# nauful/NLZM

Hardware: AMD Instinct MI355X
Metric: compress MB/s (higher is better)
Workload: dtype u8; 1 GPU; enwik9 stand-in: 1000000000 B stream, -window:28; step = 41 launches of 8 chunks (40136704 B) of the stream; timed: bytes [200683520, 401367040) of 1000000000 (a prefix: the steps asked for end before the stream does); window_bits=28, batch_chunks=8, whole_stream=False

## Files before the change

nlzm_amd/csrc/nlzm_hip.cpp:

```cpp
#include <hip/hip_runtime.h>
#include <dirent.h>
#include <unistd.h>

#include <stdarg.h>
#include <stdint.h>
#include <stdio.h>
#include <stdlib.h>
#include <string.h>

#include <array>
#include <mutex>
#include <thread>
#include <chrono>
#include <algorithm>
#include <vector>

#include "../../include/nlzm_hip.h"
#include "nlzm_core.h"
#include "nlzm_v2.h"

namespace nlzm {
void launch_rk_hash(const uint8_t *in, unsigned long long n, unsigned long long pos0, unsigned long long pos1,
                    uint32_t *out, hipStream_t st);
void launch_pipeline2(const Geom &g, const Globals &G, const v2::GlobalsV2 &V, uint32_t c0, uint32_t c1, uint32_t worker_blocks, hipStream_t st);
// ... 653 lines not shown
    if (finished) *finished = C.next_chunk >= g.nchunks;
    return 0;
}

void stage_report(const Persist &P)
{
    const double n = (double)(P.cnt.positions ? P.cnt.positions : 1);
    fprintf(stderr, "cycles/position  finder: total %.0f wait %.0f (%.0f of it for worker results) | table: total %.0f wait %.0f | parser: total %.0f wait %.0f (block set-up %.0f, passes %.0f, emit %.0f)\n",
            P.prof[17] / n, P.prof[16] / n, P.prof[25] / n, P.prof[19] / n, P.prof[18] / n, P.prof[21] / n, P.prof[20] / n, P.prof[23] / n, P.prof[24] / n, P.prof[22] / n);
    fprintf(stderr, "finder: %llu blocks (%.1f positions each); cut by: nice %llu, new top entry %llu, RK candidate %llu, RK catch-up %llu, same worker bin %llu, other %llu\n",
            P.prof[0], n / (double)(P.prof[0] ? P.prof[0] : 1), P.prof[1], P.prof[2], P.prof[3], P.prof[4], P.prof[12], P.prof[5]);
    fprintf(stderr, "table: %llu blocks, %llu on the slow path; parser: %llu blocks (%.1f nodes each), %.2f passes per block (%.0f cycles per pass), mask fills %llu, probe rounds %llu, re-sampled %llu\n",
            P.prof[6], P.prof[7], P.prof[8], n / (double)(P.prof[8] ? P.prof[8] : 1), (double)P.prof[13] / (double)(P.prof[8] ? P.prof[8] : 1),
            (double)P.prof[24] / (double)(P.prof[13] ? P.prof[13] : 1), P.prof[9], P.prof[10], P.prof[11]);
    fprintf(stderr, "table: %llu launches with %u-entry fronts on %u waves (the others: %u on %u), the shape changed %llu times\n", P.prof[114], v2::kFrCapWide, v2::kTWWide, v2::kFrCap, v2::kTW, P.prof[113]);
    fprintf(stderr, "table: blocks in which some position's front had more than 8 / 12 / 16 / 20 / 24 / the launch's capacity of entries at some step of the scan: %.2f / %.2f / %.2f / %.3f / %.3f / %.3f %%\n",
            100.0 * P.prof[105] / (P.prof[6] ? P.prof[6] : 1), 100.0 * P.prof[106] / (P.prof[6] ? P.prof[6] : 1), 100.0 * P.prof[107] / (P.prof[6] ? P.prof[6] : 1),
            100.0 * P.prof[108] / (P.prof[6] ? P.prof[6] : 1), 100.0 * P.prof[109] / (P.prof[6] ? P.prof[6] : 1), 100.0 * P.prof[7] / (P.prof[6] ? P.prof[6] : 1));
    fprintf(stderr, "finder: RK256 entries cut short by the uint16 length parameter that became the growing top entry: %llu; that ended exactly where another entry ends: %llu (%llu of them the nearer one)\n",
            P.prof[115], P.prof[116], P.prof[117]);
    fprintf(stderr, "finder: starts of nice regions whose segment the stage knew itself, ahead of the parser's word: %llu; that it had to wait for: %llu\n", P.prof[118], P.prof[119]);
    fprintf(stderr, "finder: worker results not there at the first look: %llu of positions whose call is the finder's decision (unc), %llu of others\n", P.prof[28], P.prof[29]);
    fprintf(stderr, "finder: blocks that had to wait for a worker result: %llu (%.0f cycles each); late results of hot bins' waves %llu, late results at lane 0 (the position the block before was cut at) %llu\n",
            P.prof[112], (double)P.prof[25] / (double)(P.prof[112] ? P.prof[112] : 1), P.prof[110], P.prof[111]);
    fprintf(stderr, "parser: waited for its record loader %llu times, the table stage %.0f positions ahead on average then\n", P.prof[26], (double)P.prof[27] / (double)(P.prof[26] ? P.prof[26] : 1));
    if (P.prof[96] || P.prof[100])
        fprintf(stderr, "helper parser: %llu jobs posted, %llu taken over (%llu nodes = %.1f %% of the positions), the parser stage waited %.0f cycles per position for it; "
                        "helper: %llu jobs seen, %llu done, %llu blocks (%.2f passes each), waited %.0f cycles per position for records\n",
                P.prof[96], P.prof[97], P.prof[98], 100.0 * P.prof[98] / n, P.prof[99] / n, P.prof[100], P.prof[101], P.prof[102],
                (double)P.prof[103] / (double)(P.prof[102] ? P.prof[102] : 1), P.prof[104] / n);
    if (P.prof[88]) fprintf(stderr, "finder sections (cycles/position, profile build): predict %.0f, own loads %.0f, HT rows %.0f, candidates + jobs %.0f, record + RK256 %.0f, "
                            "BT4 results (wait included) %.0f, verify %.0f, commit %.0f\n", P.prof[88] / n, P.prof[89] / n, P.prof[90] / n, P.prof[91] / n, P.prof[92] / n,
                            P.prof[93] / n, P.prof[94] / n, P.prof[95] / n);
    if (P.prof[44]) fprintf(stderr, "table stage sections (cycles/position summed over the waves, profile build): gather %.0f, scan %.0f, waiting for the carry %.0f, carry merge (the part in block order) %.0f, records %.0f\n",
                            P.prof[44] / n, P.prof[45] / n, P.prof[47] / n, P.prof[46] / n, P.prof[55] / n);
    if (P.prof[32]) {
        const double np = (double)(P.prof[13] ? P.prof[13] : 1);
        fprintf(stderr, "parser, cycles per pass (profile build): relax waves %.0f %.0f %.0f, probe wave %.0f (of it: sets that changed %.0f, mask fills %.0f), update %.0f, "
                        "barrier waits per wave %.0f %.0f %.0f %.0f; block end %.0f cycles/position\n",
                P.prof[32] / np, P.prof[33] / np, P.prof[34] / np, P.prof[35] / np, P.prof[43] / np, P.prof[41] / np, P.prof[40] / np,
                P.prof[36] / np, P.prof[37] / np, P.prof[38] / np, P.prof[39] / np, P.prof[42] / n);
        fprintf(stderr, "parser, cycles per pass by wave 0..7 (profile build): work");
        for (int w = 0; w < 8; w++) fprintf(stderr, " %.0f", P.prof[64 + w] / np);
        fprintf(stderr, " | barrier wait");
        for (int w = 0; w < 8; w++) fprintf(stderr, " %.0f", P.prof[72 + w] / np);
        fprintf(stderr, " | update");
        for (int w = 0; w < 8; w++) fprintf(stderr, " %.0f", P.prof[80 + w] / np);
        fprintf(stderr, "\n");
        const double nbk = (double)(P.prof[8] ? P.prof[8] : 1);
        fprintf(stderr, "parser loader wave, cycles per block set-up: block size + barrier %.0f, re-list %.0f, own edges %.0f, all edges %.0f, literal scan + clear + barrier %.0f\n",
                P.prof[56] / nbk, P.prof[57] / nbk, P.prof[58] / nbk, P.prof[59] / nbk, P.prof[60] / nbk);
        fprintf(stderr, "parser wave 0, cycles per pass: relax %.0f, probe %.0f, clear %.0f | update: keys + cost scan %.0f, membership %.0f, winner sets %.0f, rest %.0f\n",
                P.prof[48] / np, P.prof[49] / np, P.prof[50] / np, P.prof[51] / np, P.prof[52] / np, P.prof[53] / np, P.prof[54] / np);
    }
}
void worker_report(const WorkerCounters &wc, bool hot)
{
    fprintf(stderr, "worker lanes: %llu calls made with their fate open (at and behind a position not decided yet), %llu decisions that took calls back, %llu calls made again for it\n",
            wc.dry_runs, wc.spec_calls, wc.spec_good);
    if (hot)
        fprintf(stderr, "hot bins (a wave each): %llu over all launches, %llu of %llu calls made by their waves\n", wc.hot_bins, wc.hot_calls, wc.bt_calls);
    if (hot && wc.hot_steps) {
            fprintf(stderr, "hot bins' waves: %llu steps (%.1f per call); the next call could not start in %.1f %% of them (a call without its stores on its way) + %.1f %% (an assumed \"skip\" behind a \"call\" still open); lanes: %llu turns spent waiting for a decision\n",
                    wc.hot_steps, (double)wc.hot_steps / (wc.hot_calls ? wc.hot_calls : 1), 100.0 * wc.hot_blocked_dry / wc.hot_steps, 100.0 * wc.hot_blocked_risky / wc.hot_steps, wc.flag_waits);
        fprintf(stderr, "hot bins' waves by the bin's positions in the launch (class: waves | calls, tests/call, entries skipped | steps, cycles/step; the profile build adds | %% of the steps: some lane tests "
                        "(tests per such step; lane-steps repeated for a held slot per step), taking back, every lane holds a call, next call may not start, no entry | idle steps with an undecided position open)\n");
// ... 1064 lines not shown
```

nlzm_amd/csrc/nlzm_v2.h:

```cpp
#pragma once

#include "nlzm_core.h"
#include "xw.h"

namespace nlzm {
namespace v2 {

constexpr uint32_t kFtRing = 1u << 14;
constexpr uint32_t kFtStride = 16;
constexpr uint32_t kTpRing = 1u << 13;
constexpr uint32_t kMaxEdges = 32;
constexpr uint32_t kTpStride = 2 + 2 + 2 * kMaxEdges;
constexpr uint32_t kTpUniq = 2, kTpEdges = 4;
constexpr uint32_t kFrontMax = 264;
constexpr uint32_t kTfStride = 2 * kFrontMax;

constexpr uint32_t kFtBt = 8u, kFtTop = 16u;
struct Hx {
    alignas(128) uint32_t f_pos;
    alignas(128) uint32_t t_pos;
    alignas(128) uint32_t t_out;
    alignas(128) uint32_t p_pos;
    alignas(128) unsigned long long p_seg;
    alignas(128) uint32_t h_job;
// ... 92 lines not shown
#ifndef NLZM_SIM
            if (xw::clock100() - t0 > 3000000000ull) {
                if (xw::lane() == 0) raise(hx, kErrTimeout * 100 + code, code == 1 ? kStFinder : (code <= 3 ? kStTable : kStParser), code, v, xw::ld_agent(w));
                return false;
            }
#else
            (void)t0; (void)code;
#endif
        }
        xw::pause();
    }
}

struct FLds {
    uint32_t ht2[4096];
    uint32_t ht3[16384 + 8];
    uint32_t stage[64 * kFtStride];
    uint32_t job[64 * 3 * 4];
    uint32_t job_len[64 * 4];
    uint32_t njobs;
    uint32_t last[8192];
    Counters cnt;
};

struct Finder {
    Geom g;
    Globals G;
    GlobalsV2 V;
    uint32_t base;
    uint32_t reach;
    uint32_t reach_d = kNone;
    uint32_t s_active, s_d, s_end, s_seen;
    uint32_t rk_from, rk_to, rk_len, rk_end;
    uint32_t rk_cut = 0;
    uint32_t prev_nice, seg_s;
    uint32_t gap_last = 0;
    uint32_t n_seg_own = 0, n_seg_wait = 0;
    uint32_t t_pos_seen;
    uint32_t err;
    uint32_t dbg_a = 0;
    unsigned long long n_pos, n_nice, n_unc, n_ht, n_rkp, n_rki, n_cmp, n_blocks, n_cut0, n_cut1, n_cut2, n_cut3, n_cut4, n_cut5;
    unsigned long long n_cmp_lane = 0;
    unsigned long long t_wait, t_wait_bt = 0, t_total;
    uint32_t n_so_top = 0, n_so_tie = 0, n_so_won = 0;
    uint32_t n_late_unc = 0, n_late_other = 0, n_late_hot = 0, n_late_first = 0, n_late_blocks = 0;
    unsigned long long t_f[8] = {};
#ifdef NLZM_PROFILE
    XW_FN unsigned long long ptick() const { return xw::tick(); }
#else
    XW_FN unsigned long long ptick() const { return 0; }
#endif

    XW_FN void fail(uint32_t code, uint32_t pos, uint32_t site = 0, uint32_t x0 = 0, uint32_t x1 = 0)
    {
        err = code;
        if (xw::lane() == 0) raise(V.hx, code, kStFinder, site, pos, x0, x1);
    }

    uint32_t pend_fpos = 0;
    uint32_t pf_a0 = kNone, pf_rkh = 0;
    unsigned long long pf_own0 = 0, pf_own1 = 0;
    uint8_t pf_unc = 0;
    XW_FN void flush_fpos()
    {
        if (!pend_fpos) return;
        xw::drain();
        if (xw::lane() == 0) xw::st_agent(&V.hx->f_pos, pend_fpos);
        pend_fpos = 0;
    }

    XW_FN void slider_look(uint32_t limit)
    {
        while (s_end == kNone && s_seen < limit) {
            const uint32_t cap = umin(limit - s_seen, 512u);
            const uint32_t l = wave_cmp(G.in, s_seen - s_d, s_seen, 0, cap);
            if (l < cap) s_end = s_seen + l; else s_seen += cap;
        }
        if (s_end == kNone && (unsigned long long)s_seen >= g.n) s_end = (uint32_t)g.n;
    }
// ... 31 lines not shown
                    const uint32_t sa = (uint32_t)(ps >> 32), cover = (uint32_t)ps;
                    const bool covered = (int32_t)(cover - (a0 + 1)) >= 0;
                    const bool own = !covered && (int32_t)(gap_last - cover) < 0 && a0 - sa < kParseMax;
                    if (covered || own) {
                        xw::after_poll();
                        seg_s = sa;
                        n_seg_own += own; n_seg_wait += spins != 0;
                        xw::trace(1, a0, seg_s, (uint32_t)ps);
                        break;
                    }
                    if ((++spins & 63u) == 0) {
                        if (xw::readfirst(xw::ld_agent(&V.hx->err))) { err = kErrInternal + 100; return 1; }
#ifndef NLZM_SIM
                        if (xw::clock100() - t0 > 3000000000ull) { fail(kErrTimeout, a0, 5, (uint32_t)ps, (uint32_t)(ps >> 32)); return 1; }
#else
                        (void)t0;
#endif
                    }
                    xw::pause();
                }
                t_wait += xw::tick() - tw;
            }
        }
        const bool call_full = in_blk && !nice_pred;
        const bool call_some = call_full || (nice_pred && ((a - seg_s) & 7u) == 0);
        const bool ht_call = call_some && avail >= 4;
        const bool rk_call = call_some && avail >= 256;

        uint32_t cut_rk = 64;
        {
            const unsigned long long rkm = xw::ballot(rk_call);
            if (rkm & 1ull) {
                const uint32_t q0 = a0 - base;
                for (uint32_t e = (rk_end | 255u) + 1; e < q0 + 256; e += 256) {
                    const uint32_t hh = xw::readfirst(G.rkhash[base + e - 256]);
                    if (i == 0) G.rk_table[hh >> g.rk_shift] = q0 | (hh << g.wbits);
                    n_rki++;
                }
                xw::drain();
            }
            const unsigned long long below = rkm & ((1ull << i) - 1);
            const uint32_t prev_end = below ? (a0 + (63u - (uint32_t)__builtin_clzll(below))) - base + 256 : rk_end;
            const bool catch_up = rk_call && i > 0 && ((prev_end | 255u) + 1) < q + 256;
            const unsigned long long cm = xw::ballot(catch_up);
            if (cm) cut_rk = (uint32_t)__builtin_ctzll(cm);
        }

        const unsigned long long f1 = ptick();
        uint32_t v4 = 0;
        unsigned long long own0 = 0, own1 = 0;
        uint32_t rkh = 0;
        bool unc = false;
        if (pf_a0 == a0) {
            if (in_blk) { own0 = pf_own0; own1 = pf_own1; v4 = (uint32_t)own0; }
            rkh = rk_call ? pf_rkh : 0u;
            unc = in_blk && G.workers && pf_unc != 0;
        } else {
            if (in_blk) { own0 = load64u(cur); own1 = load64u(cur + 8); v4 = (uint32_t)own0; }
            rkh = rk_call ? G.rkhash[a] : 0u;
            unc = in_blk && G.workers && G.unc[bi] != 0;
        }
        uint32_t rkv = rk_call ? G.rk_table[rkh >> g.rk_shift] : 0u;
        const bool bt_call = call_full && avail >= 4 && G.workers;

        const unsigned long long f2 = ptick();
        const uint32_t h2 = hash4(v4 & 0xFFFFu), h3 = hash4(v4 & 0xFFFFFFu);
        const uint32_t i2 = h2 >> 20, i3 = h3 >> g.ht3_shift;
        const uint32_t tag2 = h2 & g.tag_mask, tag3 = h3 & g.tag_mask;
        const uint32_t e2 = q | (tag2 << g.wbits), e3 = q | (tag3 << g.wbits);
        uint32_t row2 = 0, r0 = 0, r1 = 0;
        if (ht_call) { row2 = L->ht2[i2]; r0 = L->ht3[i3]; r1 = L->ht3[i3 + 1]; }
        const unsigned long long htm = xw::ballot(ht_call);
        bool later = false;
        {
            uint32_t *last = L->last;
            if (ht_call) { xw::lds_max(&last[i2], i + 1); xw::lds_max(&last[4096 + (i3 & 4095u)], i + 1); }
            xw::wave_sync();
            if (ht_call) later = last[i2] > i + 1 || last[4096 + (i3 & 4095u)] > i + 1 || last[4096 + ((i3 + 1) & 4095u)] > i + 1 || last[4096 + ((i3 - 1) & 4095u)] > i + 1;
            xw::wave_sync();
            if (ht_call) { last[i2] = 0; last[4096 + (i3 & 4095u)] = 0; }
        }
        const unsigned long long dep = xw::ballot(later);
        for (unsigned long long mm = dep; mm; mm &= mm - 1) {
            const uint32_t j = (uint32_t)__builtin_ctzll(mm);
            const uint32_t b2 = xw::readlane(i2, j), b3 = xw::readlane(i3, j);
            const uint32_t x2 = xw::readlane(e2, j), x3 = xw::readlane(e3, j), y0 = xw::readlane(r0, j);
            if (ht_call && i > j) {
                if (i2 == b2) row2 = x2;
                if (i3 == b3) { r0 = x3; r1 = y0; }
                else if (i3 == b3 + 1) r0 = y0;
                else if (i3 + 1 == b3) r1 = x3;
            }
        }

        const unsigned long long f3 = ptick();
        uint32_t cd[4] = { 0, 0, 0, 0 };
        if (ht_call) {
            const uint32_t s0 = row2 & g.wmask, s1 = r0 & g.wmask, s2 = r1 & g.wmask;
            if ((row2 >> g.wbits) == tag2 && s0 < q && q - s0 <= g.wmask) cd[0] = q - s0;
            if ((r0 >> g.wbits) == tag3 && s1 < q && q - s1 <= g.wmask) cd[1] = q - s1;
            if ((r1 >> g.wbits) == tag3 && s2 < q && q - s2 <= g.wmask) cd[2] = q - s2;
        }
        const bool rk_act = rk_len > 0 && q - rk_to < rk_len;
        const uint32_t rk_eff = rk_act ? rk_len : 0u;
        const bool rk_probe = rk_call && rk_eff < 256;
        bool rk_cand = false;
        uint32_t rk_d = 0;
        if (rk_probe) {
            const uint32_t sp = rkv & g.wmask;
            if ((rkv >> g.wbits) == (rkh & g.tag_mask) && sp < q && q - sp <= g.wmask) { rk_cand = true; rk_d = q - sp; }
        }
        uint32_t rk_l16 = 16;
        if (rk_cand) {
            const unsigned long long x0 = load64u(cur - rk_d) ^ own0;
            if (x0) rk_l16 = (uint32_t)__builtin_ctzll(x0) >> 3;
            else {
                const unsigned long long x1 = load64u(cur - rk_d + 8) ^ own1;
                rk_l16 = x1 ? 8 + ((uint32_t)__builtin_ctzll(x1) >> 3) : 16;
            }
        }
        const bool rk_short = rk_cand && rk_l16 < 16 && rk_l16 < (avail & 0xFFFFu);
        const bool rk_dropped = rk_short && !(rk_l16 >= rk_eff && rk_l16 >= match_min(rk_d));
        uint32_t cl[3] = { 0, 0, 0 };
        L->njobs = 0;
        xw::wave_sync();
        unsigned long long cx0[3], cx1[3];
#pragma unroll
        for (int k = 0; k < 3; k++) {
// ... 181 lines not shown
                    so_top = so_free && (so_end > umax(before, ec) || so_win);
                    stm = xw::ballot(so_top);
                    js = stm ? (uint32_t)__builtin_ctzll(stm) : 64u;
                    const unsigned long long bad = xw::ballot(in_blk && nice_real != nice_pred);
                    cut_nice = bad ? (uint32_t)__builtin_ctzll(bad) : 64u;
                    om = xw::ballot(in_blk && od != kNone && (!s_sliding || od < s_d));
                    jo = om ? (uint32_t)__builtin_ctzll(om) : 64u;
                    m = umin(n, umin(cut_nice, umin(jo + 1 > 64 ? 64u : jo + 1, umin(cut_ev, umin(cut_rk, umin(cut_slot, cut_bin))))));
                    m = umin(m, js + 1 > 64 ? 64u : js + 1);
                    if (unc && avail >= 4 && !told && i < umin(F, m)) { xw::st_agent(G.bt_flag + bi, nice_real ? kFlagSkip : kFlagCall); told = true; }
                    if (m <= F) break;
                    if (i == F && unc) xw::st_agent(G.bt_flag + bi, kFlagCall);
                }
                if ((++spins & 63u) == 0) {
                    if (xw::readfirst(xw::ld_agent(&V.hx->err))) { err = kErrInternal + 100; return 1; }
#ifndef NLZM_SIM
                    if (xw::clock100() - t0 > 3000000000ull) {
                        const uint32_t fl = (uint32_t)__builtin_ctzll(missing | (1ull << 63));
                        fail(kErrTimeout, a0 + fl, 6, (uint32_t)__builtin_popcountll(missing) | (xw::readlane(unc ? 1u : 0u, fl) << 8) | (n << 16),
                             xw::readlane((hash4(v4) >> g.bt_shift) % G.nheads, fl));
                        return 1;
                    }
#else
                    (void)t0;
#endif
                }
                xw::pause();
            }
            if (waits) { t_wait += xw::tick() - tw; t_wait_bt += xw::tick() - tw; }
        }

        const unsigned long long f6 = ptick();
        if (m == 0) { fail(kErrInternal, a0, 7); return 1; }
        n_blocks++;
        if (m < n) {
            const uint32_t w = m == cut_nice ? 0u : (m == jo + 1 ? 1u : (m == cut_ev ? 2u : (m == cut_rk ? 3u : (m == cut_bin ? 5u : 4u))));
            n_cut0 += w == 0; n_cut1 += w == 1; n_cut2 += w == 2; n_cut3 += w == 3; n_cut4 += w == 4; n_cut5 += w == 5;
        }
        const bool fin = i < m;
        {
            const unsigned long long gapm = xw::ballot(fin && umax(before, s_sliding ? s_e : 0u) <= a);
            if (gapm) gap_last = a0 + (63u - (uint32_t)__builtin_clzll(gapm));
        }
        if (stm || xw::any(so_tie)) {
            n_so_top += (uint32_t)__builtin_popcountll(xw::ballot(fin && so_top)); n_so_tie += (uint32_t)__builtin_popcountll(xw::ballot(fin && so_tie));
            n_so_won += (uint32_t)__builtin_popcountll(xw::ballot(fin && so_win));
        }

        if (xw::any(fin && nice_real && !unc && avail >= 4 && G.workers)) { fail(kErrV2Promise, a0, 8); return 1; }

        const unsigned long long f7 = ptick();
        for (unsigned long long mm = dep & htm & ((m < 64 ? (1ull << m) : 0ull) - 1ull); mm; mm &= mm - 1) {
            const uint32_t j = (uint32_t)__builtin_ctzll(mm);
            if (i == j) { L->ht2[i2] = e2; L->ht3[i3] = e3; L->ht3[i3 + 1] = r0; }
            xw::wave_sync();
        }
        if (ht_call && i < m && !later) { L->ht2[i2] = e2; L->ht3[i3] = e3; L->ht3[i3 + 1] = r0; }
        xw::wave_sync();
        if (fin && unc && avail >= 4) xw::st_agent(G.bt_flag + bi, nice_real ? kFlagSkip : kFlagCall);
        if (fin && rk_call && (q & 255u) == 0) G.rk_table[rkh >> g.rk_shift] = q | (rkh << g.wbits);
        if (fin) {
            uint32_t w0 = np | (bt_call && bt_n ? kFtBt : 0u) | ((uint32_t)(uint8_t)own0 << 8);
            if (i == jc && s_active && s_end > a + 1) { st[2 + 2 * np] = s_d; st[3 + 2 * np] = s_end - a; np++; w0++; }
            if (s_sliding && i <= jo) { st[14] = s_d; st[15] = cap; w0 |= kFtTop; }
            if (i == jo) { st[14] = od; st[15] = cap; w0 |= kFtTop; }
            st[0] = w0; st[1] = a;
            uint32_t *dst = V.ft + (unsigned long long)(a & (kFtRing - 1)) * kFtStride;
#pragma unroll
            for (int k = 0; k < 4; k++) xw::st_agent128(dst + 4 * k, st[4 * k], st[4 * k + 1], st[4 * k + 2], st[4 * k + 3]);
        }
        {
            const uint32_t last = m - 1;
            const uint32_t pm_last = xw::readlane(pm, last);
            if (pm_last >= reach && pm_last) {
                uint32_t dm = pm_last == reach ? reach_d : kNone;
                const uint32_t le = umax(ec, so_end), ld = umin(ec == le ? ec_d : kNone, so_end == le ? so_d : kNone);
                for (unsigned long long mm = xw::ballot(fin && le == pm_last); mm; mm &= mm - 1) dm = umin(dm, xw::readlane(ld, (uint32_t)__builtin_ctzll(mm)));
                reach = pm_last; reach_d = dm;
            }
            if (s_active && jc <= last) {
                if (s_end > reach) { reach = s_end; reach_d = s_d; } else if (s_end == reach) reach_d = umin(reach_d, s_d);
                s_active = 0;
            }
            if (jo == last) { s_active = 1; s_d = xw::readlane(od, last); s_end = kNone; s_seen = a0 + last + xw::readlane(cap, last); }
            else if (js == last) { s_active = 1; s_d = xw::readlane(so_d, last); s_end = kNone; s_seen = xw::readlane(so_end, last); }
            prev_nice = xw::readlane(nice_real ? 1u : 0u, last);
            const unsigned long long rkf = xw::ballot(fin && rk_call);
            if (rkf) rk_end = (a0 + (63u - (uint32_t)__builtin_clzll(rkf))) - base + 256;
            if (rk_len && xw::any(fin && rk_call && !rk_act)) rk_len = 0;
            if (ev_ok && cut_ev == m) {
                rk_from = (a0 + last - base) - ev_d; rk_to = a0 + last - base; rk_len = ev_l; rk_cut = ev_cut ? 1u : 0u;
            }
        }
        n_pos += m;
        n_nice += (unsigned long long)__builtin_popcountll(xw::ballot(fin && nice_real));
        n_unc += (unsigned long long)__builtin_popcountll(xw::ballot(fin && unc && avail >= 4));
        n_ht += (unsigned long long)__builtin_popcountll(xw::ballot(fin && ht_call));
        n_rkp += (unsigned long long)__builtin_popcountll(xw::ballot(fin && rk_probe));
        n_rki += (unsigned long long)__builtin_popcountll(xw::ballot(fin && rk_call && (q & 255u) == 0));
        n_cmp_lane += fin ? cmpb : 0u;
        pend_fpos = a0 + m;
        pf_a0 = kNone;
        if (a0 + m < a1) {
            pf_a0 = a0 + m;
            const uint32_t na = pf_a0 + i;
            const bool nin = na < a1;
            pf_own0 = nin ? load64u(G.in + na) : 0ull; pf_own1 = nin ? load64u(G.in + na + 8) : 0ull;
            pf_rkh = (nin && la_end - na >= 256) ? G.rkhash[na] : 0u;
            pf_unc = (nin && G.workers) ? G.unc[(unsigned long long)(na - G.batch_a0)] : (uint8_t)0;
        }
        xw::trace(2, a0, n, m, reach, s_active, s_d, s_end);
        {
            const unsigned long long f8 = ptick();
            t_f[0] += f1 - f0; t_f[1] += f2 - f1; t_f[2] += f3 - f2; t_f[3] += f4 - f3; t_f[4] += f5 - f4; t_f[5] += f6 - f5; t_f[6] += f7 - f6; t_f[7] += f8 - f7;
        }
        return m;
    }

    XW_FN void run(uint32_t c0, uint32_t c1)
    {
        FLds *L = xw::lds<FLds>();
        Persist *P = G.persist;
        StateV2 *S = (StateV2 *)V.state;
        const uint32_t i = xw::lane();
        const uint32_t ht3_rows = (1u << (32 - g.ht3_shift)) + 1;
        for (uint32_t k = i; k < 8192; k += 64) L->last[k] = 0;
        for (uint32_t k = i; k < 4096; k += 64) L->ht2[k] = G.ht2[k];
        for (uint32_t k = i; k < ht3_rows; k += 64) L->ht3[k] = G.ht3[k];
        base = xw::readfirst((uint32_t)P->reb_base);
        reach = xw::readfirst(S->reach); reach_d = xw::readfirst(S->reach_d); s_active = xw::readfirst(S->s_active); s_d = xw::readfirst(S->s_d);
        s_end = xw::readfirst(S->s_end); s_seen = xw::readfirst(S->s_seen);
        prev_nice = xw::readfirst(S->prev_nice); seg_s = xw::readfirst(S->seg_s);
        rk_from = xw::readfirst(P->rk_from); rk_to = xw::readfirst(P->rk_to); rk_len = xw::readfirst(P->rk_len); rk_end = xw::readfirst(P->rk_end);
        rk_cut = rk_len >> 31; rk_len &= 0x7FFFFFFFu;
        err = xw::readfirst(P->error);
        if (!err && G.test_fail) fail(kErrInternal + 50, (uint32_t)((unsigned long long)c0 * g.chunk_size), 9);
        n_pos = n_nice = n_unc = n_ht = n_rkp = n_rki = n_cmp = n_blocks = 0;
        n_cut0 = n_cut1 = n_cut2 = n_cut3 = n_cut4 = n_cut5 = 0;
        t_wait = 0;
        const unsigned long long t_start = xw::tick();
        t_pos_seen = (uint32_t)((unsigned long long)c0 * g.chunk_size);
        unsigned long long shifts = 0;
        xw::wave_sync();
        for (uint32_t ci = c0; ci < c1 && !err; ci++) {
            const unsigned long long chunk_abs = (unsigned long long)ci * g.chunk_size;
            const unsigned long long remain = g.n - chunk_abs;
            const uint32_t chunk_read = (uint32_t)(remain < g.feed ? remain : g.feed);
            const uint32_t p_end = umin(g.chunk_size, chunk_read);
            if (chunk_abs - base >= 2ull * (g.wmask + 1)) {
                base += g.wmask + 1;
                shifts++;
                if (i == 0) { L->ht2[0] = kNone; L->ht3[0] = kNone; }
                if (rk_end >= g.wmask + 1) rk_end -= g.wmask + 1; else rk_end = 0;
                xw::wave_sync();
            }
            if (prev_nice) seg_s = (uint32_t)chunk_abs;
            gap_last = (uint32_t)chunk_abs;
            const uint32_t a1 = (uint32_t)chunk_abs + p_end, la_end = (uint32_t)chunk_abs + chunk_read;
            uint32_t a = (uint32_t)chunk_abs;
            while (a < a1 && !err) {
                const uint32_t n = umin(64u, a1 - a);
                dbg_a = a;
                if ((int32_t)(a + n - t_pos_seen - kFtRing) > 0) {
                    flush_fpos();
                    const unsigned long long tw = xw::tick();
                    if (!wait_word_ge(&V.hx->t_pos, a + n - kFtRing, V.hx, 1)) { err = kErrInternal + 100; break; }
                    t_pos_seen = xw::readfirst(xw::ld_agent(&V.hx->t_pos));
                    t_wait += xw::tick() - tw;
                }
                a += block(a, n, a1, la_end);
            }
        }
        flush_fpos();
        for (uint32_t d = 32; d; d >>= 1) n_cmp_lane += xw::shfl64(n_cmp_lane, i ^ d);
        n_cmp += xw::readfirst64(n_cmp_lane);
        xw::wave_sync();
        for (uint32_t k = xw::opaque(i); k < 4096; k += 64) G.ht2[k] = L->ht2[k];
        for (uint32_t k = xw::opaque(i); k < ht3_rows; k += 64) G.ht3[k] = L->ht3[k];
        if (i == 0) {
            P->reb_base = base;
            P->rk_from = rk_from; P->rk_to = rk_to; P->rk_len = rk_len | (rk_cut << 31); P->rk_end = rk_end;
            S->reach = reach; S->reach_d = reach_d; S->s_active = s_active; S->s_d = s_d; S->s_end = s_end; S->s_seen = s_seen;
            S->prev_nice = prev_nice; S->seg_s = seg_s;
            Counters &c = P->cnt;
            xw::atomic_add64_agent(&c.positions, n_pos); xw::atomic_add64_agent(&c.nice_positions, n_nice);
            xw::atomic_add64_agent(&c.uncertain_positions, n_unc); xw::atomic_add64_agent(&c.ht_rows, 3 * n_ht);
            xw::atomic_add64_agent(&c.rk_probes, n_rkp); xw::atomic_add64_agent(&c.rk_inserts, n_rki);
            xw::atomic_add64_agent(&c.cmp_bytes, n_cmp); xw::atomic_add64_agent(&c.shifts, shifts);
            unsigned long long *pr = P->prof;
            xw::atomic_add64_agent(&pr[0], n_blocks); xw::atomic_add64_agent(&pr[1], n_cut0); xw::atomic_add64_agent(&pr[2], n_cut1);
            xw::atomic_add64_agent(&pr[3], n_cut2); xw::atomic_add64_agent(&pr[4], n_cut3); xw::atomic_add64_agent(&pr[5], n_cut4);
            xw::atomic_add64_agent(&pr[12], n_cut5);
            xw::atomic_add64_agent(&pr[16], t_wait); xw::atomic_add64_agent(&pr[17], xw::tick() - t_start); xw::atomic_add64_agent(&pr[25], t_wait_bt);
            xw::atomic_add64_agent(&pr[28], n_late_unc); xw::atomic_add64_agent(&pr[29], n_late_other);
            xw::atomic_add64_agent(&pr[115], n_so_top); xw::atomic_add64_agent(&pr[116], n_so_tie); xw::atomic_add64_agent(&pr[117], n_so_won);
            xw::atomic_add64_agent(&pr[118], n_seg_own); xw::atomic_add64_agent(&pr[119], n_seg_wait);
            xw::atomic_add64_agent(&pr[110], n_late_hot); xw::atomic_add64_agent(&pr[111], n_late_first); xw::atomic_add64_agent(&pr[112], n_late_blocks);
#ifdef NLZM_PROFILE
            for (int z = 0; z < 8; z++) xw::atomic_add64_agent(&pr[88 + z], t_f[z]);
#endif
            if (err || xw::ld_agent(&V.hx->err)) {
                uint32_t *d = V.hx->dbg[0];
                xw::st_agent(d + 0, dbg_a); xw::st_agent(d + 1, reach); xw::st_agent(d + 2, s_active); xw::st_agent(d + 3, s_d);
                xw::st_agent(d + 4, s_end); xw::st_agent(d + 5, prev_nice); xw::st_agent(d + 6, seg_s); xw::st_agent(d + 7, rk_len);
                xw::st_agent(d + 8, t_pos_seen); xw::st_agent(d + 9, err); xw::st_agent(d + 10, base);
            }
        }
    }
};


#ifndef NLZM_FRCAP
#define NLZM_FRCAP 16
#endif
#ifndef NLZM_KTW
#define NLZM_KTW 7
#endif
#ifndef NLZM_FRCAP_WIDE
#define NLZM_FRCAP_WIDE 24
#endif
#ifndef NLZM_KTW_WIDE
#define NLZM_KTW_WIDE 5
#endif
constexpr uint32_t kFrCap = NLZM_FRCAP, kFrCapWide = NLZM_FRCAP_WIDE;
constexpr uint32_t kTW = NLZM_KTW, kTWWide = NLZM_KTW_WIDE;
constexpr uint32_t kTWMax = kTW > kTWWide ? kTW : kTWWide;
constexpr uint32_t kFrArena = (kTW * kFrCap > kTWWide * kFrCapWide ? kTW * kFrCap : kTWWide * kFrCapWide) * 2 * 64;
constexpr uint32_t kTbWidenShift = 6, kTbNarrowShift = 9;
NLZM_HD uint32_t table_waves(uint32_t wide) { return wide ? kTWWide : kTW; }
struct TWave {
    uint32_t recs[64 * kFtStride];
    uint32_t overflow;
// ... 1556 lines not shown
```

nlzm_amd/csrc/xw.h:

```cpp
#pragma once

#include <stdint.h>

#ifndef NLZM_SIM
#include <hip/hip_runtime.h>
#define XW_FN __device__ __forceinline__
#define XW_NOINLINE __device__ __noinline__

namespace xw {

XW_FN uint32_t lane() { return threadIdx.x & 63u; }
XW_FN uint32_t wave() { return (uint32_t)__builtin_amdgcn_readfirstlane((int)(threadIdx.x >> 6)); }
XW_FN uint32_t thread() { return threadIdx.x; }
XW_FN unsigned long long ballot(bool p) { return __ballot(p); }
XW_FN bool any(bool p) { return __ballot(p) != 0; }
XW_FN uint32_t readlane(uint32_t v, uint32_t l) { return (uint32_t)__builtin_amdgcn_readlane((int)v, (int)l); }
XW_FN uint32_t readfirst(uint32_t v) { return (uint32_t)__builtin_amdgcn_readfirstlane((int)v); }
XW_FN unsigned long long readlane64(unsigned long long v, uint32_t l)
{
    return ((unsigned long long)readlane((uint32_t)(v >> 32), l) << 32) | readlane((uint32_t)v, l);
}
XW_FN unsigned long long readfirst64(unsigned long long v)
{
    return ((unsigned long long)readfirst((uint32_t)(v >> 32)) << 32) | readfirst((uint32_t)v);
// ... 62 lines not shown
    u4 v;
    asm volatile("global_load_dwordx4 %0, %1, off sc1\n\ts_waitcnt vmcnt(0)" : "=v"(v) : "v"((const __attribute__((address_space(1))) uint32_t *)p) : "memory");
    return u32x4{ v.x, v.y, v.z, v.w };
}
XW_FN void atomic_or_agent(uint32_t *p, uint32_t v) { (void)__hip_atomic_fetch_or(p, v, __ATOMIC_RELAXED, __HIP_MEMORY_SCOPE_AGENT); }
XW_FN void atomic_add64_agent(unsigned long long *p, unsigned long long v) { (void)__hip_atomic_fetch_add(p, v, __ATOMIC_RELAXED, __HIP_MEMORY_SCOPE_AGENT); }
XW_FN uint32_t cas_agent(uint32_t *p, uint32_t expect, uint32_t v)
{
    (void)__hip_atomic_compare_exchange_strong(p, &expect, v, __ATOMIC_RELAXED, __ATOMIC_RELAXED, __HIP_MEMORY_SCOPE_AGENT);
    return expect;
}
XW_FN void acquire_agent() { __builtin_amdgcn_fence(__ATOMIC_ACQUIRE, "agent"); }
XW_FN void after_poll() { asm volatile("" ::: "memory"); __builtin_amdgcn_fence(__ATOMIC_ACQUIRE, "wavefront"); }
XW_FN void lds_min64(unsigned long long *p, unsigned long long v)
{
    (void)__hip_atomic_fetch_min(p, v, __ATOMIC_RELAXED, __HIP_MEMORY_SCOPE_WORKGROUP);
}
XW_FN void lds_add64(unsigned long long *p, unsigned long long v)
{
    (void)__hip_atomic_fetch_add(p, v, __ATOMIC_RELAXED, __HIP_MEMORY_SCOPE_WORKGROUP);
}
XW_FN void lds_or(uint32_t *p, uint32_t v) { (void)__hip_atomic_fetch_or(p, v, __ATOMIC_RELAXED, __HIP_MEMORY_SCOPE_WORKGROUP); }
XW_FN uint32_t lds_inc(uint32_t *p) { return __hip_atomic_fetch_add(p, 1u, __ATOMIC_RELAXED, __HIP_MEMORY_SCOPE_WORKGROUP); }
XW_FN void lds_add(uint32_t *p, uint32_t v) { (void)__hip_atomic_fetch_add(p, v, __ATOMIC_RELAXED, __HIP_MEMORY_SCOPE_WORKGROUP); }
XW_FN void lds_max(uint32_t *p, uint32_t v) { (void)__hip_atomic_fetch_max(p, v, __ATOMIC_RELAXED, __HIP_MEMORY_SCOPE_WORKGROUP); }
XW_FN void lds_st(uint32_t *p, uint32_t v) { __hip_atomic_store(p, v, __ATOMIC_RELAXED, __HIP_MEMORY_SCOPE_WORKGROUP); }
XW_FN uint32_t lds_ld(const uint32_t *p) { return __hip_atomic_load(p, __ATOMIC_RELAXED, __HIP_MEMORY_SCOPE_WORKGROUP); }
XW_FN uint32_t opaque(uint32_t v) { asm volatile("" : "+v"(v)); return v; }
XW_FN unsigned long long clock100() { return wall_clock64(); }
XW_FN unsigned long long tick() { return __builtin_readcyclecounter(); }
XW_FN void need_bt(void *, uint32_t) {}
XW_FN void trace(int, uint32_t = 0, uint32_t = 0, uint32_t = 0, uint32_t = 0, uint32_t = 0, uint32_t = 0, uint32_t = 0) {}
XW_FN uint32_t test_cut(uint32_t n) { return n; }
template <class T> XW_FN T *lds();

}

#else
#include <stdio.h>
#include <stdlib.h>
#include <string.h>
#define XW_FN inline
#define XW_NOINLINE

namespace xw {

enum : int { kReady = 0, kColl = 1, kPause = 2, kBarrier = 3, kDone = 4 };
enum : int { cBallot = 1, cReadlane = 2, cShfl = 3, cSync = 4 };

struct Fiber {
    void *sp = nullptr;
    char *stack = nullptr;
    int state = kReady;
    int coll = 0;
    unsigned long long in = 0, out = 0;
    uint32_t src = 0;
};
struct Block;
struct Wave {
    Fiber f[64];
    Block *blk = nullptr;
    uint32_t index = 0;
    bool done = false, at_barrier = false;
    unsigned long long colls = 0;
};
struct Block {
// ... 48 lines not shown
inline uint32_t scan_add(uint32_t v) { for (uint32_t d = 1; d < 64; d <<= 1) { const uint32_t o = shfl_up(v, d); if (lane() >= d) v += o; } return v; }
inline uint32_t lane_below(uint32_t v, uint32_t fill) { const uint32_t o = shfl_up(v, 1); return lane() ? o : fill; }
inline void wave_sync() { (void)collective(cSync, 0, 0); }
inline void drain() {}
inline void block_sync() { yield_to_sched(kBarrier); }
inline void pause() { yield_to_sched(kPause); }
inline void pause_long() { yield_to_sched(kPause); }
inline void st_agent(uint32_t *p, uint32_t v) { *p = v; }
inline uint32_t ld_agent(const uint32_t *p) { return *(volatile const uint32_t *)p; }
inline void st_agent64(unsigned long long *p, unsigned long long v) { *p = v; }
inline unsigned long long ld_agent64(const unsigned long long *p) { return *(volatile const unsigned long long *)p; }
inline void st_agent128(uint32_t *p, uint32_t a, uint32_t b, uint32_t c, uint32_t d) { p[0] = a; p[1] = b; p[2] = c; p[3] = d; }
struct u32x4 { uint32_t x, y, z, w; };
inline u32x4 ld_agent128(const uint32_t *p) { const volatile uint32_t *q = p; return u32x4{ q[0], q[1], q[2], q[3] }; }
inline void atomic_or_agent(uint32_t *p, uint32_t v) { *p |= v; }
inline void atomic_add64_agent(unsigned long long *p, unsigned long long v) { *p += v; }
inline uint32_t cas_agent(uint32_t *p, uint32_t expect, uint32_t v) { const uint32_t o = *p; if (o == expect) *p = v; return o; }
inline void acquire_agent() {}
inline void after_poll() {}
inline void lds_min64(unsigned long long *p, unsigned long long v) { if (v < *p) *p = v; }
inline void lds_add64(unsigned long long *p, unsigned long long v) { *p += v; }
inline void lds_or(uint32_t *p, uint32_t v) { *p |= v; }
inline uint32_t lds_inc(uint32_t *p) { return (*p)++; }
inline void lds_add(uint32_t *p, uint32_t v) { *p += v; }
inline void lds_max(uint32_t *p, uint32_t v) { if (v > *p) *p = v; }
inline void lds_st(uint32_t *p, uint32_t v) { *p = v; }
inline uint32_t lds_ld(const uint32_t *p) { return *(volatile const uint32_t *)p; }
inline uint32_t opaque(uint32_t v) { return v; }
inline unsigned long long clock100() { return sim().now; }
inline unsigned long long tick() { return sim().now; }
void need_bt(void *user, uint32_t a);
void trace(int what, uint32_t a = 0, uint32_t b = 0, uint32_t c = 0, uint32_t d = 0, uint32_t e = 0, uint32_t f = 0, uint32_t g = 0);
uint32_t test_cut(uint32_t n);
template <class T> inline T *lds() { return (T *)sim().cw->blk->lds; }

void launch(uint32_t nblocks, uint32_t nthreads, const unsigned long long *lds_bytes, void (*entry)(void *), void *arg);

}
#endif
```

Measured before the change: 6.634 MB/s.

## Parallelize HT row forwarding and commit in finder, defer counter reductions

Replaces the serial per-dependent-lane readlane loop for hash-table row forwarding with per-lane source computation followed by shuffles, resolving chained r0 dependencies through a ballot loop. When no dependent lane falls past the cut, all rows are committed in a single step using overwrite masks instead of one wave_sync per lane. Per-block ballot/popcount statistics become per-lane counters that are reduced once at the end, the next-block prefetch is issued earlier, and the drain after RK table inserts is deferred. These changes target serialized wave-level loops on the finder's critical path, at the cost of extra logic that has to match the old ordering.

After: 6.311 MB/s. 0.951x the previous value.

```diff
diff --git a/nlzm_amd/csrc/nlzm_hip.cpp b/nlzm_amd/csrc/nlzm_hip.cpp
--- a/nlzm_amd/csrc/nlzm_hip.cpp
+++ b/nlzm_amd/csrc/nlzm_hip.cpp
@@ -709,6 +709,9 @@
     if (P.prof[88]) fprintf(stderr, "finder sections (cycles/position, profile build): predict %.0f, own loads %.0f, HT rows %.0f, candidates + jobs %.0f, record + RK256 %.0f, "
                             "BT4 results (wait included) %.0f, verify %.0f, commit %.0f\n", P.prof[88] / n, P.prof[89] / n, P.prof[90] / n, P.prof[91] / n, P.prof[92] / n,
                             P.prof[93] / n, P.prof[94] / n, P.prof[95] / n);
+    fprintf(stderr, "finder: blocks with lanes that have a later lane on their HT rows: %llu committed those rows at once, %llu in order (a cut in front of one of them)\n", P.prof[123], P.prof[124]);
+    if (P.prof[88]) fprintf(stderr, "finder, lanes with a later lane on their HT rows (profile build): %.1f per block; cycles/position of the loops over them alone: forwarding (in HT rows) %.1f, "
+                            "ordered commit (in commit) %.1f\n", (double)P.prof[122] / (double)(P.prof[0] ? P.prof[0] : 1), P.prof[120] / n, P.prof[121] / n);
     if (P.prof[44]) fprintf(stderr, "table stage sections (cycles/position summed over the waves, profile build): gather %.0f, scan %.0f, waiting for the carry %.0f, carry merge (the part in block order) %.0f, records %.0f\n",
                             P.prof[44] / n, P.prof[45] / n, P.prof[47] / n, P.prof[46] / n, P.prof[55] / n);
     if (P.prof[32]) {
diff --git a/nlzm_amd/csrc/nlzm_v2.h b/nlzm_amd/csrc/nlzm_v2.h
--- a/nlzm_amd/csrc/nlzm_v2.h
+++ b/nlzm_amd/csrc/nlzm_v2.h
@@ -148,6 +148,7 @@
     uint32_t reach_d = kNone;
     uint32_t s_active, s_d, s_end, s_seen;
     uint32_t rk_from, rk_to, rk_len, rk_end;
+    uint32_t rk_stored = 0;
     uint32_t rk_cut = 0;
     uint32_t prev_nice, seg_s;
     uint32_t gap_last = 0;
@@ -157,10 +158,13 @@
     uint32_t dbg_a = 0;
     unsigned long long n_pos, n_nice, n_unc, n_ht, n_rkp, n_rki, n_cmp, n_blocks, n_cut0, n_cut1, n_cut2, n_cut3, n_cut4, n_cut5;
     unsigned long long n_cmp_lane = 0;
+    uint32_t l_nice = 0, l_unc = 0, l_ht = 0, l_rkp = 0, l_rki = 0, l_so_top = 0, l_so_tie = 0, l_so_won = 0;
+    uint32_t n_commit_par = 0, n_commit_ord = 0;
     unsigned long long t_wait, t_wait_bt = 0, t_total;
     uint32_t n_so_top = 0, n_so_tie = 0, n_so_won = 0;
     uint32_t n_late_unc = 0, n_late_other = 0, n_late_hot = 0, n_late_first = 0, n_late_blocks = 0;
     unsigned long long t_f[8] = {};
+    unsigned long long t_dep_fwd = 0, t_dep_commit = 0, n_dep = 0;
 #ifdef NLZM_PROFILE
     XW_FN unsigned long long ptick() const { return xw::tick(); }
 #else
@@ -258,13 +262,16 @@
             const unsigned long long rkm = xw::ballot(rk_call);
             if (rkm & 1ull) {
                 const uint32_t q0 = a0 - base;
+                bool inserted = false;
                 for (uint32_t e = (rk_end | 255u) + 1; e < q0 + 256; e += 256) {
                     const uint32_t hh = xw::readfirst(G.rkhash[base + e - 256]);
                     if (i == 0) G.rk_table[hh >> g.rk_shift] = q0 | (hh << g.wbits);
                     n_rki++;
-                }
-                xw::drain();
-            }
+                    inserted = true;
+                }
+                rk_stored |= inserted ? 1u : 0u;
+            }
+            if (rk_stored) { xw::drain(); rk_stored = 0; }
             const unsigned long long below = rkm & ((1ull << i) - 1);
             const uint32_t prev_end = below ? (a0 + (63u - (uint32_t)__builtin_clzll(below))) - base + 256 : rk_end;
             const bool catch_up = rk_call && i > 0 && ((prev_end | 255u) + 1) < q + 256;
@@ -307,19 +314,42 @@
             if (ht_call) { last[i2] = 0; last[4096 + (i3 & 4095u)] = 0; }
         }
         const unsigned long long dep = xw::ballot(later);
+        const unsigned long long fd0 = ptick();
+        constexpr uint32_t kNoSrc = 0xFFFFFFFFu, kSrcR0 = 64u;
+        uint32_t src2 = kNoSrc, src0 = kNoSrc, src1 = kNoSrc;
+        bool ow2 = false, ow0 = false, ow1 = false;
+        const uint32_t bb = i2 | (i3 << 12);
         for (unsigned long long mm = dep; mm; mm &= mm - 1) {
             const uint32_t j = (uint32_t)__builtin_ctzll(mm);
-            const uint32_t b2 = xw::readlane(i2, j), b3 = xw::readlane(i3, j);
-            const uint32_t x2 = xw::readlane(e2, j), x3 = xw::readlane(e3, j), y0 = xw::readlane(r0, j);
-            if (ht_call && i > j) {
-                if (i2 == b2) row2 = x2;
-                if (i3 == b3) { r0 = x3; r1 = y0; }
-                else if (i3 == b3 + 1) r0 = y0;
-                else if (i3 + 1 == b3) r1 = x3;
-            }
+            const uint32_t b = xw::readlane(bb, j);
+            const uint32_t b2 = b & 4095u, b3 = b >> 12;
+            const bool c2 = i2 == b2, cs = i3 == b3, cp = i3 == b3 + 1, cm = i3 + 1 == b3;
+            if (i > j) {
+                if (c2) src2 = j;
+                if (cs) { src0 = j; src1 = j | kSrcR0; }
+                else if (cp) src0 = j | kSrcR0;
+                else if (cm) src1 = j;
+            } else if (i < j) { ow2 |= c2; ow0 |= cs || cp; ow1 |= cs || cm; }
+        }
+        if (dep) {
+            const uint32_t g2 = xw::shfl(e2, src2 & 63u), g0 = xw::shfl(e3, src0 & 63u), g1 = xw::shfl(e3, src1 & 63u);
+            if (ht_call && src2 != kNoSrc) row2 = g2;
+            bool open0 = ht_call && src0 != kNoSrc && (src0 & kSrcR0);
+            if (ht_call && src0 != kNoSrc && !(src0 & kSrcR0)) r0 = g0;
+            for (;;) {
+                const unsigned long long om0 = xw::ballot(open0);
+                if (!om0) break;
+                const uint32_t v = xw::shfl(r0, src0 & 63u);
+                if (open0 && !((om0 >> (src0 & 63u)) & 1ull)) { r0 = v; open0 = false; }
+            }
+            const uint32_t h1 = xw::shfl(r0, src1 & 63u);
+            if (ht_call && src1 != kNoSrc) r1 = (src1 & kSrcR0) ? h1 : g1;
         }
 
         const unsigned long long f3 = ptick();
+#ifdef NLZM_PROFILE
+        t_dep_fwd += f3 - fd0; n_dep += (unsigned long long)__builtin_popcountll(dep & htm);
+#endif
         uint32_t cd[4] = { 0, 0, 0, 0 };
         if (ht_call) {
             const uint32_t s0 = row2 & g.wmask, s1 = r0 & g.wmask, s2 = r1 & g.wmask;
@@ -567,6 +597,15 @@
 
         const unsigned long long f6 = ptick();
         if (m == 0) { fail(kErrInternal, a0, 7); return 1; }
+        pf_a0 = kNone;
+        if (a0 + m < a1) {
+            pf_a0 = a0 + m;
+            const uint32_t na = pf_a0 + i;
+            const bool nin = na < a1;
+            pf_own0 = nin ? load64u(G.in + na) : 0ull; pf_own1 = nin ? load64u(G.in + na + 8) : 0ull;
+            pf_rkh = (nin && la_end - na >= 256) ? G.rkhash[na] : 0u;
+            pf_unc = (nin && G.workers) ? G.unc[(unsigned long long)(na - G.batch_a0)] : (uint8_t)0;
+        }
         n_blocks++;
         if (m < n) {
             const uint32_t w = m == cut_nice ? 0u : (m == jo + 1 ? 1u : (m == cut_ev ? 2u : (m == cut_rk ? 3u : (m == cut_bin ? 5u : 4u))));
@@ -577,23 +616,39 @@
             const unsigned long long gapm = xw::ballot(fin && umax(before, s_sliding ? s_e : 0u) <= a);
             if (gapm) gap_last = a0 + (63u - (uint32_t)__builtin_clzll(gapm));
         }
-        if (stm || xw::any(so_tie)) {
-            n_so_top += (uint32_t)__builtin_popcountll(xw::ballot(fin && so_top)); n_so_tie += (uint32_t)__builtin_popcountll(xw::ballot(fin && so_tie));
-            n_so_won += (uint32_t)__builtin_popcountll(xw::ballot(fin && so_win));
-        }
+        l_so_top += fin && so_top; l_so_tie += fin && so_tie; l_so_won += fin && so_win;
 
         if (xw::any(fin && nice_real && !unc && avail >= 4 && G.workers)) { fail(kErrV2Promise, a0, 8); return 1; }
 
         const unsigned long long f7 = ptick();
-        for (unsigned long long mm = dep & htm & ((m < 64 ? (1ull << m) : 0ull) - 1ull); mm; mm &= mm - 1) {
-            const uint32_t j = (uint32_t)__builtin_ctzll(mm);
-            if (i == j) { L->ht2[i2] = e2; L->ht3[i3] = e3; L->ht3[i3 + 1] = r0; }
+        const unsigned long long fin_m = (m < 64 ? (1ull << m) : 0ull) - 1ull;
+        if (dep & ~fin_m) {
+            for (unsigned long long mm = dep & htm & fin_m; mm; mm &= mm - 1) {
+                const uint32_t j = (uint32_t)__builtin_ctzll(mm);
+                if (i == j) { L->ht2[i2] = e2; L->ht3[i3] = e3; L->ht3[i3 + 1] = r0; }
+                xw::wave_sync();
+            }
+            n_commit_ord++;
+        } else if (dep) {
+            if (later && !ow2) L->ht2[i2] = e2;
+            if (later && !ow0) L->ht3[i3] = e3;
+            if (later && !ow1) L->ht3[i3 + 1] = r0;
+            n_commit_par++;
+#ifdef NLZM_SIM
             xw::wave_sync();
-        }
+            if (later && ((!ow2 && L->ht2[i2] != e2) || (!ow0 && L->ht3[i3] != e3) || (!ow1 && L->ht3[i3 + 1] != r0))) xw::count(3, true);
+            xw::wave_sync();
+#endif
+        }
+        xw::count(dep ? ((dep & ~fin_m) ? 1 : 0) : 2);
+#ifdef NLZM_PROFILE
+        t_dep_commit += ptick() - f7;
+#endif
         if (ht_call && i < m && !later) { L->ht2[i2] = e2; L->ht3[i3] = e3; L->ht3[i3 + 1] = r0; }
         xw::wave_sync();
         if (fin && unc && avail >= 4) xw::st_agent(G.bt_flag + bi, nice_real ? kFlagSkip : kFlagCall);
         if (fin && rk_call && (q & 255u) == 0) G.rk_table[rkh >> g.rk_shift] = q | (rkh << g.wbits);
+        if (xw::any(fin && rk_call && (q & 255u) == 0)) rk_stored = 1;
         if (fin) {
             uint32_t w0 = np | (bt_call && bt_n ? kFtBt : 0u) | ((uint32_t)(uint8_t)own0 << 8);
             if (i == jc && s_active && s_end > a + 1) { st[2 + 2 * np] = s_d; st[3 + 2 * np] = s_end - a; np++; w0++; }
@@ -628,22 +683,10 @@
             }
         }
         n_pos += m;
-        n_nice += (unsigned long long)__builtin_popcountll(xw::ballot(fin && nice_real));
-        n_unc += (unsigned long long)__builtin_popcountll(xw::ballot(fin && unc && avail >= 4));
-        n_ht += (unsigned long long)__builtin_popcountll(xw::ballot(fin && ht_call));
-        n_rkp += (unsigned long long)__builtin_popcountll(xw::ballot(fin && rk_probe));
-        n_rki += (unsigned long long)__builtin_popcountll(xw::ballot(fin && rk_call && (q & 255u) == 0));
+        l_nice += fin && nice_real; l_unc += fin && unc && avail >= 4; l_ht += fin && ht_call; l_rkp += fin && rk_probe;
+        l_rki += fin && rk_call && (q & 255u) == 0;
         n_cmp_lane += fin ? cmpb : 0u;
         pend_fpos = a0 + m;
-        pf_a0 = kNone;
-        if (a0 + m < a1) {
-            pf_a0 = a0 + m;
-            const uint32_t na = pf_a0 + i;
-            const bool nin = na < a1;
-            pf_own0 = nin ? load64u(G.in + na) : 0ull; pf_own1 = nin ? load64u(G.in + na + 8) : 0ull;
-            pf_rkh = (nin && la_end - na >= 256) ? G.rkhash[na] : 0u;
-            pf_unc = (nin && G.workers) ? G.unc[(unsigned long long)(na - G.batch_a0)] : (uint8_t)0;
-        }
         xw::trace(2, a0, n, m, reach, s_active, s_d, s_end);
         {
             const unsigned long long f8 = ptick();
@@ -709,6 +752,12 @@
         flush_fpos();
         for (uint32_t d = 32; d; d >>= 1) n_cmp_lane += xw::shfl64(n_cmp_lane, i ^ d);
         n_cmp += xw::readfirst64(n_cmp_lane);
+        for (uint32_t d = 32; d; d >>= 1) {
+            l_nice += xw::shfl(l_nice, i ^ d); l_unc += xw::shfl(l_unc, i ^ d); l_ht += xw::shfl(l_ht, i ^ d); l_rkp += xw::shfl(l_rkp, i ^ d);
+            l_rki += xw::shfl(l_rki, i ^ d); l_so_top += xw::shfl(l_so_top, i ^ d); l_so_tie += xw::shfl(l_so_tie, i ^ d); l_so_won += xw::shfl(l_so_won, i ^ d);
+        }
+        n_nice += xw::readfirst(l_nice); n_unc += xw::readfirst(l_unc); n_ht += xw::readfirst(l_ht); n_rkp += xw::readfirst(l_rkp); n_rki += xw::readfirst(l_rki);
+        n_so_top += xw::readfirst(l_so_top); n_so_tie += xw::readfirst(l_so_tie); n_so_won += xw::readfirst(l_so_won);
         xw::wave_sync();
         for (uint32_t k = xw::opaque(i); k < 4096; k += 64) G.ht2[k] = L->ht2[k];
         for (uint32_t k = xw::opaque(i); k < ht3_rows; k += 64) G.ht3[k] = L->ht3[k];
@@ -730,9 +779,11 @@
             xw::atomic_add64_agent(&pr[28], n_late_unc); xw::atomic_add64_agent(&pr[29], n_late_other);
             xw::atomic_add64_agent(&pr[115], n_so_top); xw::atomic_add64_agent(&pr[116], n_so_tie); xw::atomic_add64_agent(&pr[117], n_so_won);
             xw::atomic_add64_agent(&pr[118], n_seg_own); xw::atomic_add64_agent(&pr[119], n_seg_wait);
+            xw::atomic_add64_agent(&pr[123], n_commit_par); xw::atomic_add64_agent(&pr[124], n_commit_ord);
             xw::atomic_add64_agent(&pr[110], n_late_hot); xw::atomic_add64_agent(&pr[111], n_late_first); xw::atomic_add64_agent(&pr[112], n_late_blocks);
 #ifdef NLZM_PROFILE
             for (int z = 0; z < 8; z++) xw::atomic_add64_agent(&pr[88 + z], t_f[z]);
+            xw::atomic_add64_agent(&pr[120], t_dep_fwd); xw::atomic_add64_agent(&pr[121], t_dep_commit); xw::atomic_add64_agent(&pr[122], n_dep);
 #endif
             if (err || xw::ld_agent(&V.hx->err)) {
                 uint32_t *d = V.hx->dbg[0];
diff --git a/nlzm_amd/csrc/xw.h b/nlzm_amd/csrc/xw.h
--- a/nlzm_amd/csrc/xw.h
+++ b/nlzm_amd/csrc/xw.h
@@ -118,6 +118,7 @@
 XW_FN void need_bt(void *, uint32_t) {}
 XW_FN void trace(int, uint32_t = 0, uint32_t = 0, uint32_t = 0, uint32_t = 0, uint32_t = 0, uint32_t = 0, uint32_t = 0) {}
 XW_FN uint32_t test_cut(uint32_t n) { return n; }
+XW_FN void count(int, bool = false) {}
 template <class T> XW_FN T *lds();
 
 }
@@ -232,6 +233,8 @@
 void need_bt(void *user, uint32_t a);
 void trace(int what, uint32_t a = 0, uint32_t b = 0, uint32_t c = 0, uint32_t d = 0, uint32_t e = 0, uint32_t f = 0, uint32_t g = 0);
 uint32_t test_cut(uint32_t n);
+inline unsigned long long path_counts[8];
+inline void count(int k, bool every_lane = false) { if (every_lane || lane() == 0) path_counts[k & 7]++; }
 template <class T> inline T *lds() { return (T *)sim().cw->blk->lds; }
 
 void launch(uint32_t nblocks, uint32_t nthreads, const unsigned long long *lds_bytes, void (*entry)(void *), void *arg);
```
